# desResLab/Synchronization-avoiding-algorithms

Measured on AMD Instinct MI355X. Metric: element_updates_per_s, higher is better.
Workload: dtype f64; 1 GPU; synthetic 25n x n x n Kuhn-tet cantilever n=19: 1028850 tets, 190400 nodes, 1 x-slab partition(s), fp64, E=1e6 nu=0.3 alpha=0.5 ramped body force, dt=1.844735e-05; exchange=none (1 partition)

## Files before the change

### synchronization_avoiding_algorithms_amd/csrc/saa_api.cpp

```cpp
#include <hip/hip_runtime.h>
#include <dlfcn.h>

#include <algorithm>
#include <climits>
#include <cmath>
#include <cstdlib>
#include <cstring>
#include <iterator>
#include <mutex>
#include <new>
#include <numeric>
#include <string>
#include <utility>
#include <vector>

#include "../../include/saa_hip.h"
#include "saa_device.h"
#include "saa_modal.h"
#include "saa_opstep.h"
#include "saa_p2.h"
#include "saa_partition.h"
#include "saa_plan.h"
#include "saa_predictor.h"
#include "saa_stress.h"
// ... 85 lines not shown
  saa::DeviceMesh mesh{};
  saa::SharedMap shared{};
  saa::StepConsts consts{};
  int ramp = 1;
  double tn = 0.0;
  DevBuf<saa::BlockDesc> blocks;
  DevBuf<int32_t> halo_ids, tag, new_to_old, sh_node, sh_slot, sh_foreign, slot_sidx;
  DevBuf<uint64_t> conn;
  DevBuf<double> xyz, mass, fext, mass_node, fext_yz;
  DevBuf<double> dbuf[3];
  DevBuf<double> scratch[4];
  int i0 = 0, in_ = 1, i1 = 2;
  double *iface = nullptr;
  bool pending = false;
  int32_t n_shared = 0, n_global_shared = 0;
  std::vector<double> host_tmp;
  void *comm = nullptr;
  int32_t comm_world = 0;
  DevBuf<double> tn3;
  hipGraphExec_t sync_graph[3] = {nullptr, nullptr, nullptr};
  hipStream_t sync_graph_stream = nullptr;
  double *sync_graph_iface = nullptr;
  bool sync_graph_off = false;
  bool sync_graph_wanted = true;
  double wait_timeout_s = 30.0;
  DevBuf<int32_t> ps_err;
  DevBuf<saa::PeerEntry> ps_entries;
  int32_t ps_lds = 0, ps_max_items = 0, ps_steps = 0;
  int64_t ps_launches = 0;
  int32_t ps_lds_peer = 0;
  bool ps_capable = false;
  bool ps_capable_predict = false;
  bool ps_enabled = true;
  hipEvent_t ps_event = nullptr;
  double *rec_traj = nullptr;
  int64_t rec_cols = 0, rec_index = 0;
  int32_t rec_every = 1;
  bool det = false;
  DevBuf<double> det_force;
  DevBuf<int64_t> det_off;
  DevBuf<int32_t> det_contrib;
  saa::DetLists detl{};
  double *ps_dbg = nullptr;
  void *peer_mem = nullptr;
  int32_t peer_world = 0;
  std::vector<void *> peer_open;
  DevBuf<int32_t> px_blk_off, px_node, px_sidx, px_nb_off, px_err;
  DevBuf<saa::PeerEntry *> px_dst;
  DevBuf<int64_t> px_pstride, px_recv;
  DevBuf<saa::PeerPushRec> px_push_rec;
  DevBuf<saa::PeerRecvRec> px_recv_rec;
  DevBuf<saa::PeerSecondRec> px_second_rec;
  DevBuf<saa::PeerMap> px_map;
  DevBuf<unsigned long long> px_holders;
  DevBuf<double> px_own, px_test;
  std::vector<double> px_expected;
  saa::PeerMap peer{};
  bool peer_ready = false;
  unsigned peer_seq = 0;
  unsigned peer_seq0 = 0;
  int64_t peer_parity_repeats = 0;
  DevBuf<saa::BlockDesc> split_blocks[3];
  int32_t split_n[3] = {0, 0, 0};
  hipStream_t split_stream[3] = {nullptr, nullptr, nullptr};
  hipEvent_t split_ev[3] = {nullptr, nullptr, nullptr}, split_fork = nullptr;
  bool split_ok = false, split_wanted = true;
// ... 192 lines not shown
}

constexpr int kMaxDevices = 64;
std::mutex g_resident_mutex;
struct ResidentDeviceState {
  int handles = 0;
  saa_solver *last = nullptr;
} g_resident[kMaxDevices];

bool persistent_census(saa_solver *s, int lds, int mode) {
  const int32_t nb = static_cast<int32_t>(s->plan.blocks.size());
  DevBuf<int32_t> counter;
  bool ok = counter.upload(std::vector<int32_t>(1, 0)) == hipSuccess;
  saa::PersistArgs a{};
  a.census = counter.p;
  a.err = s->ps_err.p;
  a.timeout_ticks = 5000000;
  a.max_items = s->ps_max_items;
  ok = ok && saa::launch_persistent_steps(s->mesh, s->threads, lds, s->stream, s->consts, a, mode) == hipSuccess;
  ok = ok && hipStreamSynchronize(s->stream) == hipSuccess;
  int32_t e = 1, seen = 0;
  ok = ok && hipMemcpy(&e, s->ps_err.p, sizeof(e), hipMemcpyDeviceToHost) == hipSuccess &&
       hipMemcpy(&seen, counter.p, sizeof(seen), hipMemcpyDeviceToHost) == hipSuccess;
  counter.release();
  if (!ok || e != 0 || seen != nb) {
    (void)hipGetLastError();
    const int32_t zero = 0;
    (void)hipMemcpy(s->ps_err.p, &zero, sizeof(zero), hipMemcpyHostToDevice);
    return false;
  }
  return true;
}

void setup_persistent(saa_solver *s) {
  s->ps_capable = false;
  if (const char *env = saa::diag_env("SAA_NO_PERSISTENT"))
    if (env[0] == '1') return;
  const saa::Plan &plan = s->plan;
  const int32_t nb = static_cast<int32_t>(plan.blocks.size());
  int32_t max_items = 1, max_halo = 1;
  for (const auto &b : plan.blocks) {
    max_items = std::max(max_items, b.n_elem);
    max_halo = std::max(max_halo, b.n_halo);
  }
  const int lds = saa::persistent_lds_bytes(plan.max_local, plan.max_owned, max_items, max_halo);
  if (lds == 0) return;
  const char *trust = saa::diag_env("SAA_RESIDENT_TRUST_GRID");
  const int max_blocks = saa::persistent_max_blocks(s->device, s->threads, lds);
  if (max_blocks <= 0 || (max_blocks < nb && !(trust && trust[0] == '1'))) return;
  const size_t n_entries = 2 * 3 * static_cast<size_t>(plan.n_nodes);
  if (s->ps_entries.alloc(n_entries) != hipSuccess || s->ps_err.upload(std::vector<int32_t>(1, 0)) != hipSuccess ||
      hipMemset(s->ps_entries.p, 0, n_entries * sizeof(saa::PeerEntry)) != hipSuccess) {
    (void)hipGetLastError();
    s->ps_entries.release();
    return;
  }
  s->ps_lds = lds;
  s->ps_max_items = max_items;
  s->ps_steps = 0;
  if (const char *env = saa::diag_env("SAA_PRESET_PS_STEPS")) s->ps_steps = static_cast<int32_t>(std::strtoul(env, nullptr, 0));
  if (hipDeviceSynchronize() != hipSuccess || !persistent_census(s, lds, 0)) {
    (void)hipGetLastError();
    s->ps_entries.release();
    return;
  }
  s->ps_capable = true;
  s->ps_capable_predict = persistent_census(s, lds, 1);
  if (s->device >= 0 && s->device < kMaxDevices && hipEventCreateWithFlags(&s->ps_event, hipEventDisableTiming) == hipSuccess) {
    std::lock_guard<std::mutex> lock(g_resident_mutex);
    ++g_resident[s->device].handles;
  } else {
    (void)hipGetLastError();
    s->ps_event = nullptr;
    s->ps_capable = s->ps_capable_predict = false;
    s->ps_entries.release();
  }
}

void retire_resident(saa_solver *s) {
  if (!s->ps_event) return;
  {
    std::lock_guard<std::mutex> lock(g_resident_mutex);
    ResidentDeviceState &d = g_resident[s->device];
    if (d.last == s) d.last = nullptr;
    --d.handles;
  }
  (void)hipEventDestroy(s->ps_event);
  s->ps_event = nullptr;
}

constexpr int32_t kPersistChunk = 1000;

int try_persistent_steps(saa_solver *s, int32_t nsteps, const double *table_dev, int64_t table_row0, double *hist_dev,
                         int64_t hist_row0, int32_t *n_done, bool peer = false) {
  *n_done = 0;
  if (s->det || !s->ps_capable || !s->ps_enabled || nsteps < kPersistMinSteps || !s->mesh.mass_node || !s->mesh.fext_yz)
    return SAA_OK;
  if (peer && s->ps_lds_peer == 0) return SAA_OK;
  if (table_dev != nullptr && !s->ps_capable_predict) return SAA_OK;
  int32_t chunk = kPersistChunk;
// ... 3 lines not shown
    int32_t n = std::min(chunk, nsteps - *n_done);
    if (nsteps - *n_done - n > 0 && nsteps - *n_done - n < kPersistMinSteps) n = nsteps - *n_done;
    if (peer && s->peer_seq > 0xffffffffu - static_cast<uint32_t>(n) - 2u) return SAA_OK;
    if (static_cast<uint32_t>(s->ps_steps) > 0x7fff0000u) {
      HIP_TRY(hipMemsetAsync(s->ps_entries.p, 0, s->ps_entries.n * sizeof(saa::PeerEntry), s->stream));
      s->ps_steps = 0;
    }
    saa::PersistArgs a{};
    a.g0 = s->dbuf[s->i0].p;
    a.g1 = s->dbuf[s->in_].p;
    a.entries = s->ps_entries.p;
    a.entry_stride = 3 * static_cast<int64_t>(s->plan.n_nodes);
    a.step_base = s->ps_steps;
    a.nsteps = n;
    a.tn0 = s->tn;
    a.ramp_on = s->ramp;
    a.max_items = s->ps_max_items;
    a.table = table_dev;
    a.hist = hist_dev ? hist_dev : (table_dev == nullptr ? s->ps_dbg : nullptr);
    a.table_row0 = table_row0 + *n_done;
    a.hist_row0 = hist_row0 + *n_done;
    a.width = 3 * static_cast<int64_t>(s->n_shared);
    a.err = s->ps_err.p;
    a.timeout_ticks = static_cast<int64_t>(timeout_s * 1e8);
    a.peer = peer ? s->px_map.p : nullptr;
    a.peer_rec_off = s->ps_lds;
    a.peer_seq_base = s->peer_seq;
    a.consts = s->consts;
    a.traj = s->rec_traj;
    a.new_to_old = s->new_to_old.p;
    a.traj_cols = s->rec_cols;
    a.step_index0 = s->rec_index;
    a.save_every = s->rec_every;
    hipError_t e = hipSuccess;
    {
      std::lock_guard<std::mutex> lock(g_resident_mutex);
      ResidentDeviceState &d = g_resident[s->device];
      const bool shared_device = d.handles > 1;
      if (shared_device && d.last != nullptr && d.last != s) e = hipStreamWaitEvent(s->stream, d.last->ps_event, 0);
      if (e == hipSuccess)
        e = saa::launch_persistent_steps(s->mesh, s->threads, peer ? s->ps_lds_peer : s->ps_lds, s->stream, s->consts, a,
                                         peer ? 2 : (table_dev != nullptr ? 1 : 0));
      if (e == hipSuccess && shared_device) {
        e = hipEventRecord(s->ps_event, s->stream);
        d.last = s;
      }
    }
    if (e != hipSuccess) {
      (void)hipGetLastError();
      s->ps_capable = s->ps_capable_predict = false;
      return SAA_OK;
    }
    s->ps_steps = static_cast<int32_t>(static_cast<uint32_t>(s->ps_steps) + static_cast<uint32_t>(n));
    ++s->ps_launches;
    if (n & 1) std::swap(s->i0, s->in_);
    for (int32_t k = 0; k < n; ++k) s->tn = s->tn + s->consts.dt;
    if (peer) s->peer_seq += static_cast<uint32_t>(n);
    s->rec_index += n;
    *n_done += n;
  }
  return SAA_OK;
}

void launch_step(saa_solver *s, double *iface, const double *table_row, double *hist_row) {
  if (s->det)
    saa::launch_det_step(s->mesh, s->detl, s->threads, s->lds_bytes, s->stream, s->dbuf[s->i0].p, s->dbuf[s->in_].p,
                         s->dbuf[s->i1].p, iface, table_row, hist_row, s->consts, false);
  else
    saa::launch_fused_step(s->mesh, s->threads, s->lds_bytes, s->stream, s->dbuf[s->i0].p, s->dbuf[s->in_].p,
                           s->dbuf[s->i1].p, iface, table_row, hist_row, s->consts);
}

void launch_force(saa_solver *s, const double *d, double *f) {
// ... 1050 lines not shown
  const int64_t width = 3 * static_cast<int64_t>(s->n_shared);
  int32_t k0 = 0;
  if (int rc = try_persistent_steps(s, nsteps, s->n_shared > 0 ? table_dev : nullptr, table_row0, hist_dev, hist_row0,
                                    &k0))
    return rc;
  for (int32_t k = k0; k < nsteps; ++k) {
    s->set_ramp();
    launch_step(s, nullptr, s->n_shared > 0 ? table_dev + (table_row0 + k) * width : nullptr,
                hist_dev ? hist_dev + (hist_row0 + k) * width : nullptr);
    s->rotate();
    s->tn = s->tn + s->consts.dt;
  }
  return check_launch();
}

int saa_halo_gather(saa_solver *s, double *row_dev) {
  if (!s || (s->n_shared > 0 && !row_dev)) return fail(SAA_E_ARG, "saa_halo_gather: null argument");
  HIP_TRY(hipSetDevice(s->device));
  saa::launch_halo_gather(s->shared, s->stream, s->dbuf[s->i0].p, row_dev);
  return check_launch();
}

int saa_halo_scatter(saa_solver *s, const double *row_dev) {
  if (!s || (s->n_shared > 0 && !row_dev)) return fail(SAA_E_ARG, "saa_halo_scatter: null argument");
  HIP_TRY(hipSetDevice(s->device));
  saa::launch_halo_overwrite(s->shared, s->stream, row_dev, s->dbuf[s->i0].p, nullptr);
  return check_launch();
}

int saa_resident_kernel_info(const saa_solver *s, int32_t *capable, int32_t *lds_bytes, int32_t *steps_per_launch) {
  if (!s) return fail(SAA_E_ARG, "saa_resident_kernel_info: null handle");
  int32_t chunk = kPersistChunk;
  if (const char *env = saa::diag_env("SAA_PERSIST_CHUNK")) chunk = std::max(kPersistMinSteps, std::atoi(env));
  if (capable) *capable = s->ps_capable && s->ps_enabled && s->mesh.mass_node && s->mesh.fext_yz ? 1 : 0;
  if (lds_bytes) *lds_bytes = s->ps_lds;
  if (steps_per_launch) *steps_per_launch = chunk;
  return SAA_OK;
}

int saa_set_recorder(saa_solver *s, double *traj_dev, int64_t n_cols, int32_t save_every, int64_t next_step_index) {
  if (!s) return fail(SAA_E_ARG, "saa_set_recorder: null handle");
  if (traj_dev && (n_cols <= 0 || save_every <= 0 || next_step_index < 0))
    return fail(SAA_E_ARG, "saa_set_recorder: bad argument");
  if (s->pending) return fail(SAA_E_STATE, "saa_set_recorder: a synchronised step is in flight");
  s->rec_traj = traj_dev;
  s->rec_cols = traj_dev ? n_cols : 0;
  s->rec_every = traj_dev ? save_every : 1;
  s->rec_index = traj_dev ? next_step_index : 0;
  return SAA_OK;
}

int saa_set_deterministic(saa_solver *s, int32_t enable) {
  if (!s) return fail(SAA_E_ARG, "saa_set_deterministic: null handle");
  if (s->pending) return fail(SAA_E_STATE, "saa_set_deterministic: a synchronised step is in flight");
  HIP_TRY(hipSetDevice(s->device));
  if (enable && !s->det_off.p) {
    const saa::Plan &plan = s->plan;
    std::vector<int64_t> off(static_cast<size_t>(plan.n_nodes) + 1, 0);
    auto each = [&](auto &&fn) {
      for (const saa::BlockDesc &b : plan.blocks)
        for (int32_t e = 0; e < b.n_elem; ++e) {
          const uint16_t *it = &plan.conn[8 * static_cast<size_t>(b.elem_off + e)];
          if (it[5] == 2) continue;
          const int slots = it[5] == 1 ? 5 : 4;
          for (int a = 0; a < slots; ++a)
            if (it[a] < b.n_owned) fn(b.node_start + it[a], (b.elem_off + e) * 8 + a);
        }
    };
    each([&](int32_t node, int32_t) { ++off[node + 1]; });
    for (int32_t i = 0; i < plan.n_nodes; ++i) off[i + 1] += off[i];
    if (plan.n_items >= (1ll << 28)) return fail(SAA_E_CAPACITY, "saa_set_deterministic: too many work items");
    std::vector<int32_t> contrib(static_cast<size_t>(off[plan.n_nodes]));
    std::vector<int64_t> cur(off.begin(), off.end() - 1);
    each([&](int32_t node, int32_t id) { contrib[cur[node]++] = id; });
    HIP_TRY(s->det_off.upload(off));
    HIP_TRY(s->det_contrib.upload(contrib.empty() ? std::vector<int32_t>(1, 0) : contrib));
    HIP_TRY(s->det_force.alloc(15 * static_cast<size_t>(std::max<int64_t>(plan.n_items, 1))));
    HIP_TRY(saa::configure_det_kernels(s->lds_bytes));
    s->detl.item_force = s->det_force.p;
    s->detl.contrib_off = s->det_off.p;
    s->detl.contrib = s->det_contrib.p;
  }
  s->det = enable != 0;
  return SAA_OK;
}

int saa_set_option(saa_solver *s, const char *name, double value) {
  if (!s || !name) return fail(SAA_E_ARG, "saa_set_option: null argument");
  const std::string key(name);
  if (key == "synced_graph") {
    s->sync_graph_wanted = value != 0.0;
    return SAA_OK;
  }
  if (key == "split_stepping") {
    s->split_wanted = value != 0.0;
    return SAA_OK;
  }
  if (key == "wait_timeout_s") {
    if (!(value > 0.0) || value > 3600.0) return fail(SAA_E_ARG, "saa_set_option: wait_timeout_s must be in (0, 3600]");
    s->wait_timeout_s = std::max(1e-7, value);
    if (s->px_map.p) {
      HIP_TRY(hipSetDevice(s->device));
      HIP_TRY(hipStreamSynchronize(s->stream));
      s->peer.timeout_ticks = static_cast<int64_t>(s->wait_timeout_s * 1e8);
      HIP_TRY(s->px_map.upload(std::vector<saa::PeerMap>(1, s->peer)));
    }
    return SAA_OK;
  }
  return fail(SAA_E_ARG, "saa_set_option: unknown option '" + key + "' (synced_graph, split_stepping, wait_timeout_s)");
}

int saa_set_resident_kernel(saa_solver *s, int32_t enable) {
  if (!s) return fail(SAA_E_ARG, "saa_set_resident_kernel: null handle");
  s->ps_enabled = enable != 0;
  return SAA_OK;
}

int saa_synchronize(saa_solver *s) {
  if (!s) return fail(SAA_E_ARG, "saa_synchronize: null handle");
  HIP_TRY(hipSetDevice(s->device));
  HIP_TRY(hipStreamSynchronize(s->stream));
  if (int rc = check_persist_error(s)) return rc;
  return check_peer_error(s);
}

int saa_time_steps(saa_solver *s, int32_t nsteps, double *elapsed_ms) {
  if (!s || !elapsed_ms || nsteps < 0) return fail(SAA_E_ARG, "saa_time_steps: bad argument");
  HIP_TRY(hipSetDevice(s->device));
  hipEvent_t a, b;
  HIP_TRY(hipEventCreate(&a));
  HIP_TRY(hipEventCreate(&b));
  HIP_TRY(hipEventRecord(a, s->stream));
  int rc = saa_step(s, nsteps);
  HIP_TRY(hipEventRecord(b, s->stream));
  HIP_TRY(hipEventSynchronize(b));
  float ms = 0.f;
  HIP_TRY(hipEventElapsedTime(&ms, a, b));
  *elapsed_ms = ms;
  (void)hipEventDestroy(a);
  (void)hipEventDestroy(b);
  return rc;
}
// ... 838 lines not shown
```

### synchronization_avoiding_algorithms_amd/csrc/saa_device.h

```cpp
#pragma once
#include <hip/hip_runtime.h>
#include <stdint.h>

#include "saa_plan.h"

namespace saa {

constexpr int32_t kTagShared = 1 << 3;
constexpr int kTagSlotShift = 8;

struct DeviceMesh {
  const BlockDesc *blocks;
  const int32_t *halo_ids;
  const uint2 *conn;
  const double *xyz;
  const double *mass;
  const double *mass_node;
  const double *fext;
  const double *fext_yz;
  const int32_t *tag;
  const int32_t *slot_sidx;
  double lambda6, mu6;
  int32_t n_blocks, n_nodes, max_local, max_owned;
};
// ... 60 lines not shown
struct PersistArgs {
  double *g0, *g1;
  PeerEntry *entries;
  int64_t entry_stride;
  int32_t step_base;
  int32_t nsteps;
  double tn0;
  int32_t ramp_on;
  int32_t max_items;
  const double *table;
  double *hist;
  int64_t table_row0, hist_row0, width;
  int32_t *err;
  int64_t timeout_ticks;
  const PeerMap *peer;
  int32_t peer_rec_off;
  uint32_t peer_seq_base;
  double *traj;
  const int32_t *new_to_old;
  int64_t traj_cols, step_index0;
  int32_t save_every;
  StepConsts consts;
  int32_t *census;
};

void launch_record_column(int n_nodes, const int32_t *new_to_old, hipStream_t st, const double *d_internal, double *traj,
                          int64_t n_cols, int64_t col);
int persistent_lds_bytes(int max_local, int max_owned, int max_items, int max_halo);
hipError_t configure_persistent_peer(int lds_bytes);
int persistent_max_blocks(int device, int threads, int lds_bytes);
hipError_t launch_persistent_steps(const DeviceMesh &m, int threads, int lds_bytes, hipStream_t st, const StepConsts &k,
                                   const PersistArgs &a, int mode);

hipError_t configure_kernels(int lds_bytes);
hipError_t configure_det_kernels(int lds_bytes);
void launch_det_step(const DeviceMesh &m, const DetLists &det, int threads, int lds_bytes, hipStream_t st, const double *d0,
                     const double *dn, double *out, double *iface, const double *table_row, double *hist_row,
                     const StepConsts &k, bool force_only);
void launch_fused_step(const DeviceMesh &m, int threads, int lds_bytes, hipStream_t st, const double *d0,
                       const double *dn, double *d1, double *iface, const double *table_row, double *hist_row,
                       const StepConsts &k, const double *tn_dev = nullptr);
void launch_set_scalar(hipStream_t st, double *p, double v);
#ifdef SAA_DIAGNOSTICS
void launch_fused_step_ablated(int variant, const DeviceMesh &m, int threads, int lds_bytes, hipStream_t st,
                               const double *d0, const double *dn, double *d1, const StepConsts &k, double *dbg);
#endif
void launch_force_only(const DeviceMesh &m, int threads, int lds_bytes, hipStream_t st, const double *d,
                       double *f);
void launch_iface_finish(const DeviceMesh &m, const SharedMap &sh, hipStream_t st, const double *d0,
                         const double *dn, double *d1, double *iface, double *hist_row, const StepConsts &k,
                         const double *tn_in = nullptr, double *tn_out = nullptr);
void launch_halo_overwrite(const SharedMap &sh, hipStream_t st, const double *row, double *d1, double *hist_row);
void launch_halo_gather(const SharedMap &sh, hipStream_t st, const double *d, double *row);
void launch_cd_update(const DeviceMesh &m, hipStream_t st, const double *f_int, const double *d0,
                      const double *dn, double *d1, const StepConsts &k);
void launch_permute(int n_nodes, const int32_t *new_to_old, hipStream_t st, const double *in, double *out);
void launch_unpermute(int n_nodes, const int32_t *new_to_old, hipStream_t st, const double *in, double *out);

}
```

### synchronization_avoiding_algorithms_amd/csrc/saa_kernels.hip

```cpp
#include <hip/hip_runtime.h>
#include <algorithm>
#include <cstddef>
#include <cstdlib>
#include <stdint.h>

#include "saa_device.h"

#ifndef SAA_LB
#define SAA_LB 1024
#endif

namespace saa {

__device__ __forceinline__ double cd_update_dof(double f_int, double f_pre, double m, double d0, double dn,
                                                const StepConsts &k) {
#pragma clang fp contract(off)
  const double f_ext = f_pre * k.ramp;
  const double a = k.dt2 * (f_ext - f_int);
  const double b = (2.0 * m) * d0;
  const double c = m * dn;
  const double d = ((k.half_dt * m) * k.alpha) * dn;
  const double num = ((a + b) - c) + d;
  const double den = m + (k.half_alpha * m) * k.dt;
  return num / den;
// ... 163 lines not shown
  if (ABLATE != 1) flush<ALL_OWNED>(acc, it.a, n_owned, fa);
  else sink += fa.x + fa.y + fa.z;
  mid();
  if (it.pair) {
    const Rec rb = load_rec(rec, it.b);
    if (ABLATE == 8) {
      t1 = stamp();
      T[2] += t1 - t0;
    }
    if (ABLATE == 7) {
      fb = add3(rb.x, rb.u);
    } else {
      Vec3 gq, gr;
      tet_b_forces(pg, rp.x, rb.x, rp.u, rb.u, lam6, mu6, fb, gq, gr);
      fq = add3(fq, gq);
      fr = add3(fr, gr);
    }
    if (ABLATE == 8) {
      t0 = stamp();
      T[3] += t0 - t1;
    }
    if (ABLATE != 1) flush<ALL_OWNED>(acc, it.b, n_owned, fb);
    else sink += fb.x + fb.y + fb.z;
  }
  if (ABLATE != 7) fp = neg_sum3(add3(fa, fb), fq, fr);
  if (ABLATE == 1) {
    sink += fp.x + fp.y + fp.z + fq.x + fq.y + fq.z + fr.x + fr.y + fr.z;
    return;
  }
  flush<ALL_OWNED>(acc, it.p, n_owned, fp);
  flush<ALL_OWNED>(acc, it.q, n_owned, fq);
  flush<ALL_OWNED>(acc, it.r, n_owned, fr);
  if (ABLATE == 8) T[4] += stamp() - t0;
}

#ifndef SAA_KPRE_OWN
#define SAA_KPRE_OWN 2
#define SAA_KPRE_HALO 2
#define SAA_KPRE_CONN 2
#endif
constexpr int kPreOwn = SAA_KPRE_OWN;
constexpr int kPreHalo = SAA_KPRE_HALO;
constexpr int kPreConn = SAA_KPRE_CONN;

typedef unsigned int u32x4 __attribute__((ext_vector_type(4)));
__device__ __forceinline__ void peer_store(PeerEntry *d, double f, unsigned seq) {
  const unsigned long long b = (unsigned long long)__double_as_longlong(f);
  const u32x4 w = {(unsigned)b, seq, (unsigned)(b >> 32), seq};
  asm volatile("global_store_dwordx4 %0, %1, off sc0 sc1" ::"v"(d), "v"(w) : "memory");
}
__device__ __forceinline__ void peer_push(const PeerMap *pm, const PeerPushRec &r, int q, int c, double f, unsigned seq) {
  const int64_t par = seq & 1u;
  const int n_nb = (r.info >> 16) & 0xff;
  if (n_nb > 0) peer_store(r.dst0 + par * r.pstride0 + c, f, seq);
  if (n_nb > 1) {
    const int e0 = pm->nb_off[q];
    for (int e = e0 + 1; e < e0 + n_nb; ++e) peer_store(pm->push_dst[e] + par * pm->push_pstride[e] + c, f, seq);
  }
}
__device__ __forceinline__ double peer_wait(const PeerMap *pm, const PeerEntry *src, unsigned seq) {
  const long long t0 = wall_clock64();
  unsigned long long lo, hi;
  while (true) {
    lo = __hip_atomic_load(&src->lo, __ATOMIC_RELAXED, __HIP_MEMORY_SCOPE_SYSTEM);
    hi = __hip_atomic_load(&src->hi, __ATOMIC_RELAXED, __HIP_MEMORY_SCOPE_SYSTEM);
    if ((unsigned)(lo >> 32) == seq && (unsigned)(hi >> 32) == seq) break;
// ... 602 lines not shown
        if (((info >> 16) & 0xff) == 2) {
          int recv1 = srl[j / 3].recv1;
          asm volatile("" : "+v"(recv1));
          const PeerEntry *in = pm->inbox + (int64_t)(pseq & 1u) * pm->parity_stride + c;
          const double own = acc[3 * n + c];
          const double va = peer_wait(pm, in + r.recv0, pseq);
          const double vb = peer_wait(pm, in + recv1, pseq);
          f = (info & kPeerInfoHighest) ? (va + vb) + own : (own + va) + vb;
        } else {
          f = peer_collect(pm, r, q, c, acc[3 * n + c], pseq);
        }
        const double u = rec[6 * n + 3 + c];
        double v = cd_update_dof(f, c == 0 ? 0.0 : fextl[n], massl[n], u, dnl[i], k);
        if (tagl[n] & (1 << c)) v = 0.0;
        if (aq->hist != nullptr) aq->hist[(aq->hist_row0 + s) * aq->width + 3 * (int64_t)r.sidx + c] = v;
        commit(i, n, c, u, v);
      }
    }
    tn = tn + k.dt;
    PSTAMP(6)
    if (PEER) load_head();
    lds_barrier();
    PSTAMP(7)
  }
#ifdef SAA_PERSIST_STAMPS
  if ((tid & 63) == 0 && ap->hist != nullptr) {
    unsigned long long *dbg = reinterpret_cast<unsigned long long *>(ap->hist) + 8 * ((size_t)blockIdx.x * (nt >> 6) + (tid >> 6));
    for (int j = 0; j < 8; ++j) dbg[j] = T[j];
  }
#endif
  if (sink == 12345.678) acc[0] = sink;
}

__global__ void __launch_bounds__(SAA_LB) det_items_kernel(DeviceMesh m, const double *__restrict__ d0,
                                                           double *__restrict__ item_force) {
  extern __shared__ __attribute__((aligned(16))) double lds[];
  const BlockDesc bd = m.blocks[blockIdx.x];
  const int tid = threadIdx.x, nt = blockDim.x;
  double *rec = lds;
  const int64_t base = 3 * (int64_t)bd.node_start;
  const int32_t *hid = m.halo_ids + bd.halo_off;
  for (int i = tid; i < 3 * bd.n_owned; i += nt) {
    const int n = i / 3, c = i - 3 * n;
    rec[6 * n + c] = m.xyz[base + i];
    rec[6 * n + 3 + c] = d0[base + i];
  }
  for (int i = tid; i < 3 * bd.n_halo; i += nt) {
    const int n = i / 3, c = i - 3 * n;
    const int64_t g = 3 * (int64_t)hid[n] + c;
    rec[6 * (bd.n_owned + n) + c] = m.xyz[g];
    rec[6 * (bd.n_owned + n) + 3 + c] = d0[g];
  }
  __syncthreads();
  for (int e = tid; e < bd.n_elem; e += nt) {
    const Item it = unpack(m.conn[bd.elem_off + e]);
    if (it.null) continue;
    const Rec rp = load_rec(rec, it.p), rq = load_rec(rec, it.q), rr = load_rec(rec, it.r), ra = load_rec(rec, it.a);
    Vec3 fa, fp, fq, fr, fb = {0, 0, 0};
    const PairShared pg = pair_shared(rp.x, rq.x, rr.x, rp.u, rq.u, rr.u);
    tet_a_forces(pg, rp.x, ra.x, rp.u, ra.u, m.lambda6, m.mu6, fa, fr, fq);
    if (it.pair) {
      const Rec rb = load_rec(rec, it.b);
      Vec3 gq, gr;
      tet_b_forces(pg, rp.x, rb.x, rp.u, rb.u, m.lambda6, m.mu6, fb, gq, gr);
      fq = add3(fq, gq);
      fr = add3(fr, gr);
// ... 206 lines not shown
  int per_cu = 0, cus = 0;
  const void *fns[3] = {reinterpret_cast<const void *>(&persistent_steps_kernel<false, false>),
                        reinterpret_cast<const void *>(&persistent_steps_kernel<true, false>),
                        reinterpret_cast<const void *>(&persistent_steps_kernel<false, true>)};
  for (const void *fn : fns)
    if (hipFuncSetAttribute(fn, hipFuncAttributeMaxDynamicSharedMemorySize, lds_bytes) != hipSuccess) return 0;
  int occ[3] = {0, 0, 0};
  if (hipOccupancyMaxActiveBlocksPerMultiprocessor(&occ[0], persistent_steps_kernel<false, false>, threads, lds_bytes) != hipSuccess ||
      hipOccupancyMaxActiveBlocksPerMultiprocessor(&occ[1], persistent_steps_kernel<true, false>, threads, lds_bytes) != hipSuccess ||
      hipOccupancyMaxActiveBlocksPerMultiprocessor(&occ[2], persistent_steps_kernel<false, true>, threads, lds_bytes) != hipSuccess)
    return 0;
  per_cu = occ[0] < occ[1] ? occ[0] : occ[1];
  per_cu = per_cu < occ[2] ? per_cu : occ[2];
  constexpr int kSgprBand = 112, kWavesPerSimd = 800 / (kSgprBand + 16) < 8 ? 800 / (kSgprBand + 16) : 8;
  const int by_sgpr = threads >= 256 ? kWavesPerSimd / (threads / 256) : kWavesPerSimd * (256 / threads);
  per_cu = per_cu < by_sgpr ? per_cu : by_sgpr;
  if (hipDeviceGetAttribute(&cus, hipDeviceAttributeMultiprocessorCount, device) != hipSuccess) return 0;
  return per_cu * cus;
}

hipError_t launch_persistent_steps(const DeviceMesh &m, int threads, int lds_bytes, hipStream_t st, const StepConsts &k,
                                   const PersistArgs &a, int mode) {
  static_assert(offsetof(PersistKernArgs, a) == sizeof(DeviceMesh) + sizeof(StepConsts) && alignof(PersistArgs) == 8,
                "kernel-argument segment: the argument block follows the mesh and the step constants without padding");
  if (mode == 1)
    hipLaunchKernelGGL((persistent_steps_kernel<true, false>), dim3(m.n_blocks), dim3(threads), lds_bytes, st, m, k, a);
  else if (mode == 2)
    hipLaunchKernelGGL((persistent_steps_kernel<false, true>), dim3(m.n_blocks), dim3(threads), lds_bytes, st, m, k, a);
  else
    hipLaunchKernelGGL((persistent_steps_kernel<false, false>), dim3(m.n_blocks), dim3(threads), lds_bytes, st, m, k, a);
  return hipGetLastError();
}

void launch_force_only(const DeviceMesh &m, int threads, int lds_bytes, hipStream_t st, const double *d,
                       double *f) {
  StepConsts k{};
  hipLaunchKernelGGL(fused_step_kernel<true>, dim3(m.n_blocks), dim3(threads), lds_bytes, st, m, d, d, f,
                     static_cast<double *>(nullptr), static_cast<const double *>(nullptr),
                     static_cast<double *>(nullptr), k, static_cast<const PeerMap *>(nullptr), 0u,
                     static_cast<const double *>(nullptr));
}

void launch_iface_finish(const DeviceMesh &m, const SharedMap &sh, hipStream_t st, const double *d0,
                         const double *dn, double *d1, double *iface, double *hist_row, const StepConsts &k,
                         const double *tn_in, double *tn_out) {
  const int n = 3 * (sh.n_shared + sh.n_foreign);
  if (n == 0 && tn_in == nullptr) return;
  hipLaunchKernelGGL(iface_finish_kernel, dim3(((n > 0 ? n : 1) + 255) / 256), dim3(256), 0, st, m, sh, d0, dn, d1, iface,
                     hist_row, k, tn_in, tn_out);
}

void launch_halo_overwrite(const SharedMap &sh, hipStream_t st, const double *row, double *d1, double *hist_row) {
  const int n = 3 * sh.n_shared;
  if (n == 0) return;
  hipLaunchKernelGGL(halo_overwrite_kernel, dim3((n + 255) / 256), dim3(256), 0, st, sh, row, d1, hist_row);
}

void launch_halo_gather(const SharedMap &sh, hipStream_t st, const double *d, double *row) {
  const int n = 3 * sh.n_shared;
  if (n == 0) return;
  hipLaunchKernelGGL(halo_gather_kernel, dim3((n + 255) / 256), dim3(256), 0, st, sh, d, row);
}

void launch_cd_update(const DeviceMesh &m, hipStream_t st, const double *f_int, const double *d0,
                      const double *dn, double *d1, const StepConsts &k) {
  const int64_t n = 3 * (int64_t)m.n_nodes;
// ... 25 lines not shown
```

### synchronization_avoiding_algorithms_amd/solver.py

```python
from __future__ import annotations

import ctypes as C

import numpy as np

from . import _lib


def _f64(a, n=None):
    a = np.ascontiguousarray(np.asarray(a, dtype=np.float64).reshape(-1))
    if n is not None and a.size != n:
        raise ValueError(f"expected {n} values, got {a.size}")
    return a


def _i32(a):
    return np.ascontiguousarray(np.asarray(a, dtype=np.int32).reshape(-1))


def _dptr(a):
    return a.ctypes.data_as(C.POINTER(C.c_double))


def _iptr(a):
# ... 33 lines not shown
            lumped_mass=_dptr(mass), f_ext=_dptr(fext), dirichlet_dofs=_iptr(dd), n_dirichlet=dd.size,
            shared_nodes=_iptr(sn), shared_slots=_iptr(ss), n_shared=sn.size,
            n_global_shared=self.n_global_shared, lambda_=float(lmd), mu=float(mu), dt=float(dt),
            alpha=float(alpha), ramp=1 if ramp else 0, device=int(device), block_nodes=int(block_nodes),
            threads=int(threads))
        _lib.check(self._lib.saa_create(C.byref(pb), C.byref(self._h)))
        self._iface = None

    def close(self):
        if getattr(self, "_h", None) is not None and self._h.value:
            self._lib.saa_destroy(self._h)
            self._h = C.c_void_p()

    def __del__(self):
        try:
            self.close()
        except Exception:
            pass

    def __enter__(self):
        return self

    def __exit__(self, *exc):
        self.close()

    def plan_stats(self) -> dict:
        st = _lib.PlanStats()
        _lib.check(self._lib.saa_plan_stats_get(self._h, C.byref(st)))
        return st.as_dict()

    def resident_kernel_info(self) -> dict:
        cap, lds, spl = C.c_int32(), C.c_int32(), C.c_int32()
        _lib.check(self._lib.saa_resident_kernel_info(self._h, C.byref(cap), C.byref(lds), C.byref(spl)))
        return {"capable": bool(cap.value), "lds_bytes": lds.value, "steps_per_launch": spl.value}

    def set_recorder(self, traj=None, save_every=1, next_step_index=0):
        if traj is None:
            _lib.check(self._lib.saa_set_recorder(self._h, None, 0, 1, 0))
            self._traj = None
            return
        if traj.dim() != 2 or traj.shape[0] != self.n_dof:
            raise ValueError(f"trajectory matrix must be ({self.n_dof}, n_cols)")
        _lib.check(self._lib.saa_set_recorder(self._h, _dev(traj), int(traj.shape[1]), int(save_every),
                                              int(next_step_index)))
        self._traj = traj

    def set_resident_kernel(self, enable: bool):
        _lib.check(self._lib.saa_set_resident_kernel(self._h, 1 if enable else 0))

    def set_option(self, name: str, value: float):
        _lib.check(self._lib.saa_set_option(self._h, name.encode(), float(value)))

    def set_deterministic(self, enable: bool):
        _lib.check(self._lib.saa_set_deterministic(self._h, 1 if enable else 0))

    def set_stream(self, stream_ptr):
        _lib.check(self._lib.saa_set_stream(self._h, C.c_void_p(int(stream_ptr) if stream_ptr else 0)))

    def synchronize(self):
        _lib.check(self._lib.saa_synchronize(self._h))

    def set_state(self, d0, dn, tn=0.0):
        a, b = _f64(d0, self.n_dof), _f64(dn, self.n_dof)
        _lib.check(self._lib.saa_set_state(self._h, _dptr(a), _dptr(b), float(tn)))

    def get_state(self):
        d0, dn, tn = np.empty(self.n_dof), np.empty(self.n_dof), C.c_double()
# ... 140 lines not shown
```

Measured before the change: 114.5 billion element-updates/s.

## Add specialized resident plain kernel with cached per-element reciprocal determinants

```diff
diff --git a/synchronization_avoiding_algorithms_amd/csrc/saa_api.cpp b/synchronization_avoiding_algorithms_amd/csrc/saa_api.cpp
--- a/synchronization_avoiding_algorithms_amd/csrc/saa_api.cpp
+++ b/synchronization_avoiding_algorithms_amd/csrc/saa_api.cpp
@@ -141,6 +141,9 @@
   bool ps_capable = false;
   bool ps_capable_predict = false;
   bool ps_enabled = true;
+  int32_t ps_plain_rdet_off = 0;
+  int32_t ps_plain_lds = 0;
+  bool ps_plain_wanted = true;
   hipEvent_t ps_event = nullptr;
   double *rec_traj = nullptr;
   int64_t rec_cols = 0, rec_index = 0;
@@ -399,8 +402,34 @@
   return true;
 }
 
+bool resident_plain_census(saa_solver *s, int lds) {
+  const int32_t nb = static_cast<int32_t>(s->plan.blocks.size());
+  DevBuf<int32_t> counter;
+  bool ok = counter.upload(std::vector<int32_t>(1, 0)) == hipSuccess;
+  saa::PlainArgs a{};
+  a.census = counter.p;
+  a.err = s->ps_err.p;
+  a.timeout_ticks = 5000000;
+  a.max_items = s->ps_max_items;
+  a.rdet_off = s->ps_plain_rdet_off;
+  ok = ok && saa::launch_resident_plain(s->mesh, s->threads, lds, s->stream, s->consts, a) == hipSuccess;
+  ok = ok && hipStreamSynchronize(s->stream) == hipSuccess;
+  int32_t e = 1, seen = 0;
+  ok = ok && hipMemcpy(&e, s->ps_err.p, sizeof(e), hipMemcpyDeviceToHost) == hipSuccess &&
+       hipMemcpy(&seen, counter.p, sizeof(seen), hipMemcpyDeviceToHost) == hipSuccess;
+  counter.release();
+  if (!ok || e != 0 || seen != nb) {
+    (void)hipGetLastError();
+    const int32_t zero = 0;
+    (void)hipMemcpy(s->ps_err.p, &zero, sizeof(zero), hipMemcpyHostToDevice);
+    return false;
+  }
+  return true;
+}
+
 void setup_persistent(saa_solver *s) {
   s->ps_capable = false;
+  s->ps_plain_lds = 0;
   if (const char *env = saa::diag_env("SAA_NO_PERSISTENT"))
     if (env[0] == '1') return;
   const saa::Plan &plan = s->plan;
@@ -433,6 +462,13 @@
   }
   s->ps_capable = true;
   s->ps_capable_predict = persistent_census(s, lds, 1);
+  {
+    const int plds = saa::resident_plain_lds_bytes(plan.max_local, plan.max_owned, max_items, max_halo);
+    s->ps_plain_rdet_off = saa::resident_plain_rdet_off(plan.max_local, plan.max_owned, max_halo);
+    if (plds > 0 && s->threads >= 128 && saa::resident_plain_max_blocks(s->device, s->threads, plds) >= nb && resident_plain_census(s, plds))
+      s->ps_plain_lds = plds;
+    (void)hipGetLastError();
+  }
   if (s->device >= 0 && s->device < kMaxDevices && hipEventCreateWithFlags(&s->ps_event, hipEventDisableTiming) == hipSuccess) {
     std::lock_guard<std::mutex> lock(g_resident_mutex);
     ++g_resident[s->device].handles;
@@ -502,13 +538,35 @@
     a.traj_cols = s->rec_cols;
     a.step_index0 = s->rec_index;
     a.save_every = s->rec_every;
+    const bool plain = !peer && table_dev == nullptr && hist_dev == nullptr && s->rec_traj == nullptr && s->ps_plain_wanted &&
+                       s->ps_plain_lds > 0;
+    saa::PlainArgs pa{};
+    if (plain) {
+      pa.g0 = a.g0;
+      pa.g1 = a.g1;
+      pa.entries = a.entries;
+      pa.entry_stride = a.entry_stride;
+      pa.step_base = a.step_base;
+      pa.nsteps = a.nsteps;
+      pa.tn0 = a.tn0;
+      pa.ramp_on = a.ramp_on;
+      pa.max_items = a.max_items;
+      pa.rdet_off = s->ps_plain_rdet_off;
+      pa.err = a.err;
+      pa.timeout_ticks = a.timeout_ticks;
+      pa.stamps = reinterpret_cast<unsigned long long *>(s->ps_dbg);
+    }
     hipError_t e = hipSuccess;
     {
       std::lock_guard<std::mutex> lock(g_resident_mutex);
       ResidentDeviceState &d = g_resident[s->device];
       const bool shared_device = d.handles > 1;
       if (shared_device && d.last != nullptr && d.last != s) e = hipStreamWaitEvent(s->stream, d.last->ps_event, 0);
-      if (e == hipSuccess)
+      if (e == hipSuccess && plain && saa::launch_resident_plain(s->mesh, s->threads, s->ps_plain_lds, s->stream, s->consts, pa) != hipSuccess) {
+        (void)hipGetLastError();
+        s->ps_plain_lds = 0;
+      }
+      if (e == hipSuccess && !(plain && s->ps_plain_lds > 0))
         e = saa::launch_persistent_steps(s->mesh, s->threads, peer ? s->ps_lds_peer : s->ps_lds, s->stream, s->consts, a,
                                          peer ? 2 : (table_dev != nullptr ? 1 : 0));
       if (e == hipSuccess && shared_device) {
@@ -1625,7 +1683,8 @@
   if (!s) return fail(SAA_E_ARG, "saa_resident_kernel_info: null handle");
   int32_t chunk = kPersistChunk;
   if (const char *env = saa::diag_env("SAA_PERSIST_CHUNK")) chunk = std::max(kPersistMinSteps, std::atoi(env));
-  if (capable) *capable = s->ps_capable && s->ps_enabled && s->mesh.mass_node && s->mesh.fext_yz ? 1 : 0;
+  if (capable)
+    *capable = s->ps_capable && s->ps_enabled && s->mesh.mass_node && s->mesh.fext_yz ? (s->ps_plain_lds > 0 && s->ps_plain_wanted ? 2 : 1) : 0;
   if (lds_bytes) *lds_bytes = s->ps_lds;
   if (steps_per_launch) *steps_per_launch = chunk;
   return SAA_OK;
@@ -1689,6 +1748,10 @@
     s->split_wanted = value != 0.0;
     return SAA_OK;
   }
+  if (key == "resident_plain") {
+    s->ps_plain_wanted = value != 0.0;
+    return SAA_OK;
+  }
   if (key == "wait_timeout_s") {
     if (!(value > 0.0) || value > 3600.0) return fail(SAA_E_ARG, "saa_set_option: wait_timeout_s must be in (0, 3600]");
     s->wait_timeout_s = std::max(1e-7, value);
@@ -1700,7 +1763,7 @@
     }
     return SAA_OK;
   }
-  return fail(SAA_E_ARG, "saa_set_option: unknown option '" + key + "' (synced_graph, split_stepping, wait_timeout_s)");
+  return fail(SAA_E_ARG, "saa_set_option: unknown option '" + key + "' (synced_graph, split_stepping, resident_plain, wait_timeout_s)");
 }
 
 int saa_set_resident_kernel(saa_solver *s, int32_t enable) {
diff --git a/synchronization_avoiding_algorithms_amd/csrc/saa_device.h b/synchronization_avoiding_algorithms_amd/csrc/saa_device.h
--- a/synchronization_avoiding_algorithms_amd/csrc/saa_device.h
+++ b/synchronization_avoiding_algorithms_amd/csrc/saa_device.h
@@ -116,6 +116,26 @@
 hipError_t launch_persistent_steps(const DeviceMesh &m, int threads, int lds_bytes, hipStream_t st, const StepConsts &k,
                                    const PersistArgs &a, int mode);
 
+struct PlainArgs {
+  double *g0, *g1;
+  PeerEntry *entries;
+  int64_t entry_stride;
+  int32_t step_base, nsteps;
+  double tn0;
+  int32_t ramp_on, max_items;
+  int32_t rdet_off;
+  int32_t reserved;
+  int32_t *err;
+  int64_t timeout_ticks;
+  int32_t *census;
+  unsigned long long *stamps;
+};
+int resident_plain_rdet_off(int max_local, int max_owned, int max_halo);
+int resident_plain_lds_bytes(int max_local, int max_owned, int max_items, int max_halo);
+int resident_plain_max_blocks(int device, int threads, int lds_bytes);
+hipError_t launch_resident_plain(const DeviceMesh &m, int threads, int lds_bytes, hipStream_t st, const StepConsts &k,
+                                 const PlainArgs &a);
+
 hipError_t configure_kernels(int lds_bytes);
 hipError_t configure_det_kernels(int lds_bytes);
 void launch_det_step(const DeviceMesh &m, const DetLists &det, int threads, int lds_bytes, hipStream_t st, const double *d0,
diff --git a/synchronization_avoiding_algorithms_amd/csrc/saa_kernels.hip b/synchronization_avoiding_algorithms_amd/csrc/saa_kernels.hip
--- a/synchronization_avoiding_algorithms_amd/csrc/saa_kernels.hip
+++ b/synchronization_avoiding_algorithms_amd/csrc/saa_kernels.hip
@@ -219,6 +219,71 @@
   flush<ALL_OWNED>(acc, it.q, n_owned, fq);
   flush<ALL_OWNED>(acc, it.r, n_owned, fr);
   if (ABLATE == 8) T[4] += stamp() - t0;
+}
+
+__device__ __forceinline__ double tet_rdet(const Vec3 &e1, const Vec3 &c1) {
+  const double det = e1.x * c1.x + e1.y * c1.y + e1.z * c1.z;
+  double r = __builtin_amdgcn_rcp(det);
+  r = __builtin_fma(r, __builtin_fma(-det, r, 1.0), r);
+  return r;
+}
+__device__ __forceinline__ void tet_core_r(const Vec3 &e1, const Vec3 &e2, const Vec3 &e3, const Vec3 &c1, const Vec3 &w1,
+                                           const Vec3 &w2, const Vec3 &w3, double r, double lam6, double mu6, Vec3 &f1,
+                                           Vec3 &f2, Vec3 &f3) {
+  const Vec3 c2 = cross(e3, e1), c3 = cross(e1, e2);
+  const double h00 = w1.x * c1.x + w2.x * c2.x + w3.x * c3.x;
+  const double h11 = w1.y * c1.y + w2.y * c2.y + w3.y * c3.y;
+  const double h22 = w1.z * c1.z + w2.z * c2.z + w3.z * c3.z;
+  const double g01 = w1.x * c1.y + w2.x * c2.y + w3.x * c3.y + w1.y * c1.x + w2.y * c2.x + w3.y * c3.x;
+  const double g02 = w1.x * c1.z + w2.x * c2.z + w3.x * c3.z + w1.z * c1.x + w2.z * c2.x + w3.z * c3.x;
+  const double g12 = w1.y * c1.z + w2.y * c2.z + w3.y * c3.z + w1.z * c1.y + w2.z * c2.y + w3.z * c3.y;
+  const double ls = lam6 * r, ms = mu6 * r, ms2 = ms + ms;
+  const double ltr = ls * (h00 + h11 + h22);
+  const double sxx = ltr + ms2 * h00, syy = ltr + ms2 * h11, szz = ltr + ms2 * h22;
+  const double syz = ms * g12, sxz = ms * g02, sxy = ms * g01;
+  f1 = {sxx * c1.x + sxy * c1.y + sxz * c1.z, sxy * c1.x + syy * c1.y + syz * c1.z,
+        sxz * c1.x + syz * c1.y + szz * c1.z};
+  f2 = {sxx * c2.x + sxy * c2.y + sxz * c2.z, sxy * c2.x + syy * c2.y + syz * c2.z,
+        sxz * c2.x + syz * c2.y + szz * c2.z};
+  f3 = {sxx * c3.x + sxy * c3.y + sxz * c3.z, sxy * c3.x + syy * c3.y + syz * c3.z,
+        sxz * c3.x + syz * c3.y + szz * c3.z};
+}
+__device__ __forceinline__ double2 item_rdet(const uint2 w, const double *rec) {
+  const Item it = unpack(w);
+  if (it.null) return {0.0, 0.0};
+  const Vec3 xp = load_rec(rec, it.p).x;
+  const Vec3 c = cross(sub(load_rec(rec, it.r).x, xp), sub(load_rec(rec, it.q).x, xp));
+  double2 rd = {tet_rdet(sub(load_rec(rec, it.a).x, xp), c), 0.0};
+  if (it.pair) rd.y = tet_rdet(sub(load_rec(rec, it.b).x, xp), {-c.x, -c.y, -c.z});
+  return rd;
+}
+template <bool ALL_OWNED, typename Hook = NoHook>
+__device__ __forceinline__ void item_forces_rdet(const uint2 w, const double2 rd, const double *rec, double *acc,
+                                                 int n_owned, double lam6, double mu6, Hook mid = Hook()) {
+  const Item it = unpack(w);
+  if (it.null) {
+    mid();
+    return;
+  }
+  const Rec rp = load_rec(rec, it.p), rq = load_rec(rec, it.q), rr = load_rec(rec, it.r);
+  const Rec ra = load_rec(rec, it.a);
+  const PairShared pg = pair_shared(rp.x, rq.x, rr.x, rp.u, rq.u, rr.u);
+  Vec3 fa, fq, fr, fb = {0, 0, 0};
+  tet_core_r(sub(ra.x, rp.x), pg.er, pg.eq, pg.c, sub(ra.u, rp.u), pg.wr, pg.wq, rd.x, lam6, mu6, fa, fr, fq);
+  flush<ALL_OWNED>(acc, it.a, n_owned, fa);
+  mid();
+  if (it.pair) {
+    const Rec rb = load_rec(rec, it.b);
+    const Vec3 nc = {-pg.c.x, -pg.c.y, -pg.c.z};
+    Vec3 gq, gr;
+    tet_core_r(sub(rb.x, rp.x), pg.eq, pg.er, nc, sub(rb.u, rp.u), pg.wq, pg.wr, rd.y, lam6, mu6, fb, gq, gr);
+    fq = add3(fq, gq);
+    fr = add3(fr, gr);
+    flush<ALL_OWNED>(acc, it.b, n_owned, fb);
+  }
+  flush<ALL_OWNED>(acc, it.p, n_owned, neg_sum3(add3(fa, fb), fq, fr));
+  flush<ALL_OWNED>(acc, it.q, n_owned, fq);
+  flush<ALL_OWNED>(acc, it.r, n_owned, fr);
 }
 
 #ifndef SAA_KPRE_OWN
@@ -887,6 +952,255 @@
   if (sink == 12345.678) acc[0] = sink;
 }
 
+struct PlainKernArgs {
+  DeviceMesh m;
+  StepConsts k;
+  PlainArgs a;
+};
+typedef const __attribute__((address_space(4))) PlainArgs *PlainArgsPtr;
+__global__ void __launch_bounds__(SAA_LB) resident_plain_kernel(DeviceMesh m, StepConsts k, PlainArgs ) {
+  extern __shared__ __attribute__((aligned(16))) double lds[];
+  PlainArgsPtr ap;
+  {
+    const __attribute__((address_space(4))) char *seg =
+        (const __attribute__((address_space(4))) char *)__builtin_amdgcn_kernarg_segment_ptr();
+    seg += offsetof(PlainKernArgs, a);
+    asm volatile("" : "+s"(seg));
+    ap = reinterpret_cast<PlainArgsPtr>(seg);
+  }
+  if (ap->census != nullptr) {
+    if (threadIdx.x == 0) {
+      int32_t *cnt = ap->census;
+      __hip_atomic_fetch_add(cnt, 1, __ATOMIC_RELAXED, __HIP_MEMORY_SCOPE_AGENT);
+      const long long t0 = wall_clock64();
+      while (__hip_atomic_load(cnt, __ATOMIC_RELAXED, __HIP_MEMORY_SCOPE_AGENT) < (int32_t)gridDim.x) {
+        if (__hip_atomic_load(ap->err, __ATOMIC_RELAXED, __HIP_MEMORY_SCOPE_SYSTEM) != 0) break;
+        if (wall_clock64() - t0 > ap->timeout_ticks) {
+          __hip_atomic_store(ap->err, 1, __ATOMIC_RELAXED, __HIP_MEMORY_SCOPE_SYSTEM);
+          break;
+        }
+        __builtin_amdgcn_s_sleep(8);
+      }
+    }
+    return;
+  }
+  struct {
+    double *g0, *g1;
+    int32_t nsteps, max_items;
+    double tn0;
+  } a = {ap->g0, ap->g1, ap->nsteps, ap->max_items, ap->tn0};
+  const int pblock = plan_block(blockIdx.x, m.n_blocks);
+  const BlockDesc bd = m.blocks[pblock];
+  const int tid = threadIdx.x, nt = blockDim.x;
+  double *rec = lds;
+  double *acc = lds + 6 * m.max_local;
+  const int o_dn = persist_off_dn(m.max_local, m.max_owned), o_mass = o_dn + 3 * m.max_owned, o_fext = o_mass + m.max_owned;
+  const int64_t base = 3 * (int64_t)bd.node_start;
+  double *dnl = lds + o_dn;
+  double *massl = lds + o_mass;
+  double *fextl = lds + o_fext;
+  const int o_tag = 2 * (o_fext + m.max_owned), o_hg = o_tag + m.max_owned;
+  int32_t *tagl = reinterpret_cast<int32_t *>(lds) + o_tag;
+  int32_t *hgl = reinterpret_cast<int32_t *>(lds) + o_hg;
+  double2 *rdl = reinterpret_cast<double2 *>(reinterpret_cast<char *>(lds) + ap->rdet_off);
+  uint2 *connl = reinterpret_cast<uint2 *>(rdl) + a.max_items;
+  const int n_own3 = 3 * bd.n_owned, n_halo3 = 3 * bd.n_halo;
+  const int32_t *hid = m.halo_ids + bd.halo_off;
+
+  {
+    constexpr int kOwnSweeps = 3, kHaloSweeps = 2;
+    int64_t hgi[kHaloSweeps];
+    int32_t hnode[kHaloSweeps];
+    double ox[kOwnSweeps], ou[kOwnSweeps], hx[kHaloSweeps], hu[kHaloSweeps];
+#pragma unroll
+    for (int j = 0; j < kHaloSweeps; ++j) hnode[j] = hid[min(tid + j * nt, max(n_halo3 - 1, 0)) / 3];
+    dma_words(a.g1 + base, dnl, 2 * n_own3, tid, nt);
+    dma_words(m.mass_node + bd.node_start, massl, 2 * bd.n_owned, tid, nt);
+    dma_words(m.fext_yz + bd.node_start, fextl, 2 * bd.n_owned, tid, nt);
+    dma_words(m.tag + bd.node_start, tagl, bd.n_owned, tid, nt);
+    dma_words(m.conn + bd.elem_off, connl, 2 * bd.n_elem, tid, nt);
+#pragma unroll
+    for (int j = 0; j < kOwnSweeps; ++j) {
+      const int i = min(tid + j * nt, n_own3 - 1);
+      ox[j] = m.xyz[base + i];
+      ou[j] = a.g0[base + i];
+    }
+#pragma unroll
+    for (int j = 0; j < kHaloSweeps; ++j) {
+      hgi[j] = 3 * (int64_t)hnode[j] + (min(tid + j * nt, max(n_halo3 - 1, 0)) % 3);
+      hx[j] = m.xyz[hgi[j]];
+      hu[j] = a.g0[hgi[j]];
+    }
+#pragma unroll
+    for (int j = 0; j < kOwnSweeps; ++j) {
+      const int i = tid + j * nt;
+      if (i < n_own3) {
+        const int n = i / 3, c = i - 3 * n;
+        rec[6 * n + c] = ox[j];
+        rec[6 * n + 3 + c] = ou[j];
+        acc[i] = 0.0;
+      }
+    }
+    for (int i = tid + kOwnSweeps * nt; i < n_own3; i += nt) {
+      const int n = i / 3, c = i - 3 * n;
+      rec[6 * n + c] = m.xyz[base + i];
+      rec[6 * n + 3 + c] = a.g0[base + i];
+      acc[i] = 0.0;
+    }
+#pragma unroll
+    for (int j = 0; j < kHaloSweeps; ++j) {
+      const int i = tid + j * nt;
+      if (i < n_halo3) {
+        const int n = i / 3, c = i - 3 * n;
+        rec[6 * (bd.n_owned + n) + c] = hx[j];
+        rec[6 * (bd.n_owned + n) + 3 + c] = hu[j];
+        hgl[i] = (int32_t)hgi[j];
+      }
+    }
+    for (int i = tid + kHaloSweeps * nt; i < n_halo3; i += nt) {
+      const int n = i / 3, c = i - 3 * n;
+      const int64_t g = 3 * (int64_t)hid[n] + c;
+      rec[6 * (bd.n_owned + n) + c] = m.xyz[g];
+      rec[6 * (bd.n_owned + n) + 3 + c] = a.g0[g];
+      hgl[i] = (int32_t)g;
+    }
+  }
+  if (tid == 0 && n_halo3 == 0) hgl[0] = 0;
+  __syncthreads();
+
+  const int n_pre = min(bd.n_interior, nt);
+  const int n_ir = bd.n_interior - n_pre, n_ir_pad = (n_ir + 63) & ~63;
+  const int n_post = n_ir_pad + (bd.n_elem - bd.n_interior);
+  auto post_item = [&](int p) { return p < n_ir_pad ? (p < n_ir ? n_pre + p : -1) : bd.n_interior + (p - n_ir_pad); };
+  double tn = a.tn0;
+  const uint2 kNullItem = {0u, 2u << 28};
+  uint2 w_first = tid < n_pre ? connl[tid] : kNullItem, w_post[2];
+  int e_post[2];
+#pragma unroll
+  for (int j = 0; j < 2; ++j) {
+    const int p = tid + j * nt;
+    e_post[j] = p < n_post ? post_item(p) : -1;
+    w_post[j] = e_post[j] >= 0 ? connl[e_post[j]] : kNullItem;
+  }
+  {
+    const double2 r0 = item_rdet(w_first, rec), r1 = item_rdet(w_post[0], rec), r2 = item_rdet(w_post[1], rec);
+    __syncthreads();
+    if (tid < n_pre) rdl[tid] = r0;
+    if (e_post[0] >= 0) rdl[e_post[0]] = r1;
+    if (e_post[1] >= 0) rdl[e_post[1]] = r2;
+  }
+  const int e_first = min(tid, a.max_items - 1);
+  e_post[0] = max(e_post[0], 0);
+  e_post[1] = max(e_post[1], 0);
+#ifdef SAA_PERSIST_STAMPS
+  unsigned long long T[8] = {0, 0, 0, 0, 0, 0, 0, 0}, tk = stamp();
+#endif
+  const int h_ramp_on = ap->ramp_on;
+  const unsigned h_step_base = (unsigned)ap->step_base;
+  const PeerEntry *h_entries = ap->entries;
+  const int64_t h_entry_stride = ap->entry_stride;
+  for (int s = 0; s < a.nsteps; ++s) {
+    k.ramp = h_ramp_on ? (tn <= 1 ? tn : 1.0) : 1.0;
+    int ltid = tid;
+    asm volatile("" : "+v"(ltid));
+    const unsigned want = h_step_base + (unsigned)s;
+    const PeerEntry *ein = h_entries + (int64_t)(s & 1) * h_entry_stride;
+    unsigned long long hlo[kPH], hhi[kPH];
+    auto fetch = [&]() {
+      if (s > 0) {
+#pragma unroll
+        for (int j = 0; j < kPH; ++j) {
+          const PeerEntry *e = ein + hgl[min(ltid + j * nt, max(n_halo3 - 1, 0))];
+          hlo[j] = __hip_atomic_load(&e->lo, __ATOMIC_RELAXED, __HIP_MEMORY_SCOPE_AGENT);
+          hhi[j] = __hip_atomic_load(&e->hi, __ATOMIC_RELAXED, __HIP_MEMORY_SCOPE_AGENT);
+        }
+      }
+    };
+    asm volatile("" : "+v"(w_first.x), "+v"(w_first.y), "+v"(w_post[0].x), "+v"(w_post[0].y), "+v"(w_post[1].x), "+v"(w_post[1].y),
+                 "+v"(e_post[0]), "+v"(e_post[1]));
+    item_forces_rdet<true>(w_first, rdl[e_first], rec, acc, bd.n_owned, m.lambda6, m.mu6, fetch);
+    PSTAMP(0)
+    PSTAMP(1)
+    if (s > 0) {
+      auto settle = [&](int i, unsigned long long lo, unsigned long long hi) {
+        if ((unsigned)(lo >> 32) != want || (unsigned)(hi >> 32) != want) {
+          const PeerEntry *e = ein + hgl[i];
+          const long long t0 = wall_clock64();
+          do {
+            int32_t *errp = *(int32_t *volatile const __attribute__((address_space(4))) *)&ap->err;
+            if (__hip_atomic_load(errp, __ATOMIC_RELAXED, __HIP_MEMORY_SCOPE_SYSTEM) != 0) break;
+            if (wall_clock64() - t0 > *(volatile const __attribute__((address_space(4))) int64_t *)&ap->timeout_ticks) {
+              __hip_atomic_store(errp, 1, __ATOMIC_RELAXED, __HIP_MEMORY_SCOPE_SYSTEM);
+              break;
+            }
+            __builtin_amdgcn_s_sleep(1);
+            lo = __hip_atomic_load(&e->lo, __ATOMIC_RELAXED, __HIP_MEMORY_SCOPE_AGENT);
+            hi = __hip_atomic_load(&e->hi, __ATOMIC_RELAXED, __HIP_MEMORY_SCOPE_AGENT);
+          } while ((unsigned)(lo >> 32) != want || (unsigned)(hi >> 32) != want);
+        }
+        return __longlong_as_double((long long)((hi << 32) | (lo & 0xffffffffull)));
+      };
+#pragma unroll
+      for (int j = 0; j < kPH; ++j) {
+        const int i = ltid + j * nt;
+        if (i < n_halo3) {
+          const int n = i / 3, c = i - 3 * n;
+          rec[6 * (bd.n_owned + n) + 3 + c] = settle(i, hlo[j], hhi[j]);
+        }
+      }
+      for (int i = ltid + kPH * nt; i < n_halo3; i += nt) {
+        const int n = i / 3, c = i - 3 * n;
+        rec[6 * (bd.n_owned + n) + 3 + c] = settle(i, 0ull, 0ull);
+      }
+    }
+    PSTAMP(2)
+    lds_barrier();
+    PSTAMP(3)
+    if (tid < n_post) item_forces_rdet<false>(w_post[0], rdl[e_post[0]], rec, acc, bd.n_owned, m.lambda6, m.mu6);
+    if (tid + nt < n_post) item_forces_rdet<false>(w_post[1], rdl[e_post[1]], rec, acc, bd.n_owned, m.lambda6, m.mu6);
+    for (int p = tid + 2 * nt; p < n_post; p += nt) {
+      const int e = post_item(p);
+      if (e >= 0) {
+        const uint2 w = connl[e];
+        item_forces_rdet<false>(w, item_rdet(w, rec), rec, acc, bd.n_owned, m.lambda6, m.mu6);
+      }
+    }
+    PSTAMP(4)
+    double *gnext = (s & 1) ? ap->g0 : ap->g1;
+    PeerEntry *eout = ap->entries + (int64_t)((s + 1) & 1) * ap->entry_stride + base;
+    const unsigned stampw = (unsigned)(ap->step_base + s + 1);
+    const bool keep = s + 2 >= ap->nsteps;
+    lds_barrier();
+    PSTAMP(5)
+    asm volatile("" : "+v"(ltid));
+    for (int i = ltid; i < n_own3; i += nt) {
+      const int n = i / 3, c = i - 3 * n;
+      const double u = rec[6 * n + 3 + c];
+      double v = cd_update_dof(acc[i], c == 0 ? 0.0 : fextl[n], massl[n], u, dnl[i], k);
+      if (tagl[n] & (1 << c)) v = 0.0;
+      if (keep) gnext[base + i] = v;
+      {
+        const unsigned long long b = (unsigned long long)__double_as_longlong(v);
+        const u32x4 w4 = {(unsigned)b, stampw, (unsigned)(b >> 32), stampw};
+        asm volatile("global_store_dwordx4 %0, %1, off sc1" ::"v"(eout + i), "v"(w4) : "memory");
+      }
+      dnl[i] = u;
+      rec[6 * n + 3 + c] = v;
+      acc[i] = 0.0;
+    }
+    tn = tn + k.dt;
+    PSTAMP(6)
+    lds_barrier();
+    PSTAMP(7)
+  }
+#ifdef SAA_PERSIST_STAMPS
+  if ((tid & 63) == 0 && ap->stamps != nullptr) {
+    unsigned long long *dbg = ap->stamps + 8 * ((size_t)blockIdx.x * (nt >> 6) + (tid >> 6));
+    for (int j = 0; j < 8; ++j) dbg[j] = T[j];
+  }
+#endif
+}
+
 __global__ void __launch_bounds__(SAA_LB) det_items_kernel(DeviceMesh m, const double *__restrict__ d0,
                                                            double *__restrict__ item_force) {
   extern __shared__ __attribute__((aligned(16))) double lds[];
@@ -1159,6 +1473,37 @@
   return hipGetLastError();
 }
 
+int resident_plain_rdet_off(int max_local, int max_owned, int max_halo) {
+  const long long bytes = 8ll * (persist_off_dn(max_local, max_owned) + 3 * max_owned + 2 * max_owned) + 4ll * max_owned +
+                          12ll * max_halo + 16;
+  return bytes <= 160 * 1024 ? (int)((bytes + 15) / 16 * 16) : 0;
+}
+int resident_plain_lds_bytes(int max_local, int max_owned, int max_items, int max_halo) {
+  const long long bytes = resident_plain_rdet_off(max_local, max_owned, max_halo) + 16ll * max_items;
+  return resident_plain_rdet_off(max_local, max_owned, max_halo) > 0 && bytes <= 160 * 1024 ? (int)bytes : 0;
+}
+
+int resident_plain_max_blocks(int device, int threads, int lds_bytes) {
+  int per_cu = 0, cus = 0;
+  if (hipFuncSetAttribute(reinterpret_cast<const void *>(&resident_plain_kernel), hipFuncAttributeMaxDynamicSharedMemorySize,
+                          lds_bytes) != hipSuccess ||
+      hipOccupancyMaxActiveBlocksPerMultiprocessor(&per_cu, resident_plain_kernel, threads, lds_bytes) != hipSuccess)
+    return 0;
+  constexpr int kSgprBand = 112, kWavesPerSimd = 800 / (kSgprBand + 16) < 8 ? 800 / (kSgprBand + 16) : 8;
+  const int by_sgpr = threads >= 256 ? kWavesPerSimd / (threads / 256) : kWavesPerSimd * (256 / threads);
+  per_cu = per_cu < by_sgpr ? per_cu : by_sgpr;
+  if (hipDeviceGetAttribute(&cus, hipDeviceAttributeMultiprocessorCount, device) != hipSuccess) return 0;
+  return per_cu * cus;
+}
+
+hipError_t launch_resident_plain(const DeviceMesh &m, int threads, int lds_bytes, hipStream_t st, const StepConsts &k,
+                                 const PlainArgs &a) {
+  static_assert(offsetof(PlainKernArgs, a) == sizeof(DeviceMesh) + sizeof(StepConsts) && alignof(PlainArgs) == 8,
+                "kernel-argument segment: the argument block follows the mesh and the step constants without padding");
+  hipLaunchKernelGGL(resident_plain_kernel, dim3(m.n_blocks), dim3(threads), lds_bytes, st, m, k, a);
+  return hipGetLastError();
+}
+
 void launch_force_only(const DeviceMesh &m, int threads, int lds_bytes, hipStream_t st, const double *d,
                        double *f) {
   StepConsts k{};
diff --git a/synchronization_avoiding_algorithms_amd/solver.py b/synchronization_avoiding_algorithms_amd/solver.py
--- a/synchronization_avoiding_algorithms_amd/solver.py
+++ b/synchronization_avoiding_algorithms_amd/solver.py
@@ -89,7 +89,8 @@
     def resident_kernel_info(self) -> dict:
         cap, lds, spl = C.c_int32(), C.c_int32(), C.c_int32()
         _lib.check(self._lib.saa_resident_kernel_info(self._h, C.byref(cap), C.byref(lds), C.byref(spl)))
-        return {"capable": bool(cap.value), "lds_bytes": lds.value, "steps_per_launch": spl.value}
+        return {"capable": bool(cap.value), "lds_bytes": lds.value, "steps_per_launch": spl.value,
+                "plain_kernel": cap.value == 2}
 
     def set_recorder(self, traj=None, save_every=1, next_step_index=0):
         if traj is None:
```

Result: no change. 114.6 billion element-updates/s, median of 2 (+0.1%).
